# knagrecha/saturn

Measured on AMD Instinct MI355X. Metric: samples_per_s, higher is better.
Workload: dtype bf16; 1 GPU; model=gptj-6b, global_batch=16, seq_len=512, parallelism=dp1, optimizer=fused_sgd

## Files before the change

### saturn_amd/models/gptj.py

```python

from __future__ import annotations


from dataclasses import dataclass

import torch
import torch.nn as nn

from saturn_amd.ops.functional import (
    fused_gelu,
    FusedLayerNorm,
    apply_rope,
    causal_attention,
    fused_add3,
    fused_cross_entropy,
    rope_tables,
    FusedDropout,
    FusedEmbedding,
)


@dataclass
class GPTJConfig:
    vocab_size: int = 50400
    n_ctx: int = 512
    n_embd: int = 4096
    n_head: int = 16
    n_layer: int = 28
    rotary_dim: int = 64
    embd_pdrop: float = 0.0
    resid_pdrop: float = 0.0


class GPTJAttention(nn.Module):
    def __init__(self, cfg: GPTJConfig):
        super().__init__()
        self.n_head = cfg.n_head
        self.head_dim = cfg.n_embd // cfg.n_head
        self.rotary_dim = cfg.rotary_dim
        E = cfg.n_embd
        self.q_proj = nn.Linear(E, E, bias=False)
        self.k_proj = nn.Linear(E, E, bias=False)
        self.v_proj = nn.Linear(E, E, bias=False)
        self.out_proj = nn.Linear(E, E, bias=False)
        self.n_ctx = cfg.n_ctx
        self._rope_f32 = rope_tables(cfg.n_ctx, cfg.rotary_dim)

    def _rope(self, device):
        if self._rope_f32[0].device != device:
            self._rope_f32 = tuple(t.to(device) for t in self._rope_f32)
        return self._rope_f32

    def forward(self, x):
        B, T, E = x.shape
        H, D = self.n_head, self.head_dim
        q = self.q_proj(x).view(B, T, H, D)
        k = self.k_proj(x).view(B, T, H, D)
        v = self.v_proj(x).view(B, T, H, D)
        cos, sin = self._rope(x.device)
        q = apply_rope(q, cos, sin)
        k = apply_rope(k, cos, sin)
        q = q.transpose(1, 2)
        k = k.transpose(1, 2)
        v = v.transpose(1, 2)
        o = causal_attention(q, k, v)
        o = o.transpose(1, 2).reshape(B, T, -1)
        return self.out_proj(o)


class GPTJMLP(nn.Module):
    def __init__(self, cfg: GPTJConfig):
        super().__init__()
        E = cfg.n_embd
        self.fc_in = nn.Linear(E, 4 * E)
        self.fc_out = nn.Linear(4 * E, E)

    def forward(self, x):
        return self.fc_out(fused_gelu(self.fc_in(x)))


class GPTJBlock(nn.Module):

    def __init__(self, cfg: GPTJConfig):
        super().__init__()
        self.ln_1 = FusedLayerNorm(cfg.n_embd)
        self.attn = GPTJAttention(cfg)
        self.mlp = GPTJMLP(cfg)
        self.drop = FusedDropout(cfg.resid_pdrop)

    def forward(self, x):
        h = self.ln_1(x)
        return fused_add3(x, self.drop(self.attn(h)), self.drop(self.mlp(h)))


class GPTJForCausalLM(nn.Module):
    def __init__(self, cfg: GPTJConfig):
        super().__init__()
        self.cfg = cfg
        self.wte = FusedEmbedding(cfg.vocab_size, cfg.n_embd)
        self.drop = FusedDropout(cfg.embd_pdrop)
        self.h = nn.ModuleList(GPTJBlock(cfg) for _ in range(cfg.n_layer))
        self.ln_f = FusedLayerNorm(cfg.n_embd)
        self.lm_head = nn.Linear(cfg.n_embd, cfg.vocab_size, bias=True)
        self.apply(self._init)

    @staticmethod
    def _init(m):
        if isinstance(m, nn.Linear):
            nn.init.normal_(m.weight, std=0.02)
            if m.bias is not None:
                nn.init.zeros_(m.bias)
        elif isinstance(m, nn.Embedding):
            nn.init.normal_(m.weight, std=0.02)

    def forward(self, input_ids):
        x = self.drop(self.wte(input_ids))
        for block in self.h:
            x = block(x)
        x = self.ln_f(x)
        return self.lm_head(x)


def pretraining_loss(logits, labels):
    return fused_cross_entropy(logits, labels, shift=True)


class _EmbedStage(nn.Module):
    def __init__(self, wte):
        super().__init__()
        self.wte = wte

    def forward(self, input_ids):
        return self.wte(input_ids)


class _HeadStage(nn.Module):
    def __init__(self, ln_f, lm_head):
        super().__init__()
        self.ln_f = ln_f
        self.lm_head = lm_head

    def forward(self, x):
        return self.lm_head(self.ln_f(x))


def as_sequential(model: GPTJForCausalLM) -> nn.Sequential:
    return nn.Sequential(
        _EmbedStage(model.wte), *model.h, _HeadStage(model.ln_f, model.lm_head)
    )


def get_gptj_model(kwargs=None):
    kwargs = kwargs or {}
    cfg = GPTJConfig(
        n_layer=kwargs.get("n_layer", 28),
        n_embd=kwargs.get("n_embd", 4096),
        n_head=kwargs.get("n_head", 16),
        n_ctx=kwargs.get("n_ctx", 512),
        vocab_size=kwargs.get("vocab_size", 50400),
        rotary_dim=kwargs.get("rotary_dim", 64),
        embd_pdrop=kwargs.get("embd_pdrop", 0.0),
        resid_pdrop=kwargs.get("resid_pdrop", 0.0),
    )
    torch.manual_seed(kwargs.get("seed", 0))
    return GPTJForCausalLM(cfg)


class SyntheticTokens(torch.utils.data.Dataset):

    def __init__(self, n: int, seq_len: int, vocab: int, seed: int = 1):
        g = torch.Generator().manual_seed(seed)
        self.data = torch.randint(0, vocab, (n, seq_len), generator=g)

    def __len__(self):
        return len(self.data)

    def __getitem__(self, i):
        return self.data[i]


def _collate(batch):
    x = torch.stack(batch)
    return x, x.clone()


def make_token_dataloader(batch_size=8, seq_len=512, vocab=50400, n_batches=64):
    def get_dataloader():
        return torch.utils.data.DataLoader(
            SyntheticTokens(batch_size * n_batches, seq_len, vocab),
            batch_size=batch_size,
            shuffle=False,
            collate_fn=_collate,
        )

    return get_dataloader
```

### saturn_amd/ops/csrc/bindings.cpp

```cpp

#include <torch/extension.h>
#include <vector>

namespace samd {
void fused_sgd(std::vector<at::Tensor> params, std::vector<at::Tensor> grads,
               std::vector<at::Tensor> moms, std::vector<at::Tensor> masters,
               double lr, double momentum, double weight_decay);
void fused_adam(std::vector<at::Tensor> params, std::vector<at::Tensor> grads,
                std::vector<at::Tensor> ms, std::vector<at::Tensor> vs,
                std::vector<at::Tensor> masters, double lr, double beta1,
                double beta2, double eps, double weight_decay, double bc1,
                double bc2);
std::vector<at::Tensor> norm_fwd(at::Tensor x, at::Tensor w,
                                 c10::optional<at::Tensor> b, double eps,
                                 bool rms);
std::vector<at::Tensor> norm_bwd(at::Tensor dy, at::Tensor x, at::Tensor w,
                                 at::Tensor mean, at::Tensor rstd, bool rms,
                                 bool needs_db);
std::vector<at::Tensor> ce_fwd(at::Tensor logits, at::Tensor targets,
                               int64_t Tr, int64_t ignore_index);
at::Tensor ce_bwd(at::Tensor logits, at::Tensor targets, at::Tensor lse,
                  at::Tensor dloss, int64_t Tr, int64_t ignore_index);
void rope_apply(at::Tensor y, at::Tensor x, at::Tensor cos_t, at::Tensor sin_t,
                int64_t t_len, int64_t t_off, bool half_style, bool backward);
at::Tensor gelu_fwd(at::Tensor x);
at::Tensor gelu_bwd(at::Tensor dy, at::Tensor x);
std::vector<at::Tensor> attn_fwd(at::Tensor q, at::Tensor k, at::Tensor v,
                                 bool causal, int64_t kv_len);
std::vector<at::Tensor> attn_bwd(at::Tensor dout, at::Tensor q, at::Tensor k,
                                 at::Tensor v, at::Tensor o, at::Tensor lse,
                                 bool causal, int64_t kv_len);
at::Tensor add3(at::Tensor a, at::Tensor b, at::Tensor c);
at::Tensor swiglu_fwd(at::Tensor gate, at::Tensor up);
std::vector<at::Tensor> swiglu_bwd(at::Tensor dout, at::Tensor gate,
                                   at::Tensor up);
at::Tensor embed_fwd(at::Tensor weight, at::Tensor idx);
at::Tensor embed_bwd(at::Tensor dout, at::Tensor idx, long vocab);
at::Tensor dropout_fwd(at::Tensor x, double p, long seed);
at::Tensor dropout_bwd(at::Tensor dout, double p, long seed);
std::vector<at::Tensor> moe_route_fwd(at::Tensor logits, int64_t top_k,
                                      at::ScalarType out_dtype);
at::Tensor moe_route_bwd(at::Tensor logits, at::Tensor ids,
                         at::Tensor dweights);
std::vector<at::Tensor> moe_sort(at::Tensor ids, int64_t n_expert);
at::Tensor moe_permute_fwd(at::Tensor x, at::Tensor order, int64_t top_k);
at::Tensor moe_permute_bwd(at::Tensor dxs, at::Tensor pos);
at::Tensor moe_combine_fwd(at::Tensor y, at::Tensor weights, at::Tensor pos);
std::vector<at::Tensor> moe_combine_bwd(at::Tensor dout, at::Tensor y,
                                        at::Tensor weights, at::Tensor pos);
}

PYBIND11_MODULE(TORCH_EXTENSION_NAME, m) {
  m.doc() = "saturn_amd hand-written CDNA4 (gfx950) kernels";
  m.def("fused_sgd", &samd::fused_sgd, "fused multi-tensor SGD");
  m.def("fused_adam", &samd::fused_adam, "fused multi-tensor AdamW");
  m.def("norm_fwd", &samd::norm_fwd, "LayerNorm/RMSNorm forward");
  m.def("norm_bwd", &samd::norm_bwd, "LayerNorm/RMSNorm backward");
  m.def("ce_fwd", &samd::ce_fwd, "fused cross-entropy forward");
  m.def("ce_bwd", &samd::ce_bwd, "fused cross-entropy backward");
  m.def("rope_apply", &samd::rope_apply,
        "fused rotary embedding (out-of-place, offset table rows)");
  m.def("gelu_fwd", &samd::gelu_fwd, "fused tanh-approx GELU forward");
  m.def("gelu_bwd", &samd::gelu_bwd, "fused tanh-approx GELU backward");
  m.def("attn_fwd", &samd::attn_fwd, "fused flash attention forward",
        py::arg("q"), py::arg("k"), py::arg("v"), py::arg("causal"),
        py::arg("kv_len") = -1);
  m.def("attn_bwd", &samd::attn_bwd, "fused flash attention backward",
        py::arg("dout"), py::arg("q"), py::arg("k"), py::arg("v"),
        py::arg("o"), py::arg("lse"), py::arg("causal"),
        py::arg("kv_len") = -1);
  m.def("add3", &samd::add3, "fused 3-way residual add");
  m.def("swiglu_fwd", &samd::swiglu_fwd, "fused silu(gate)*up");
  m.def("swiglu_bwd", &samd::swiglu_bwd, "fused SwiGLU backward");
  m.def("embed_fwd", &samd::embed_fwd, "token embedding gather");
  m.def("embed_bwd", &samd::embed_bwd, "embedding scatter-add backward");
  m.def("dropout_fwd", &samd::dropout_fwd, "counter-based fused dropout");
  m.def("dropout_bwd", &samd::dropout_bwd, "dropout backward (mask recompute)");
  m.def("moe_route_fwd", &samd::moe_route_fwd,
        "MoE softmax + top-k + renormalise (ties to the lower expert)");
  m.def("moe_route_bwd", &samd::moe_route_bwd, "MoE routing backward");
  m.def("moe_sort", &samd::moe_sort,
        "stable counting sort of (token, slot) pairs by expert");
  m.def("moe_permute_fwd", &samd::moe_permute_fwd,
        "gather token rows into expert order");
  m.def("moe_permute_bwd", &samd::moe_permute_bwd,
        "sum each token's k permuted rows");
  m.def("moe_combine_fwd", &samd::moe_combine_fwd,
        "weighted sum of each token's k expert rows");
  m.def("moe_combine_bwd", &samd::moe_combine_bwd,
        "combine backward: dy and fp32 dweights");
}
```

### saturn_amd/ops/csrc/gelu.hip

```cpp

#include <torch/extension.h>
#include <ATen/hip/HIPContext.h>

#include "common.h"

namespace samd {

typedef __attribute__((ext_vector_type(8))) short short8v_g;

__device__ __forceinline__ float tanh_fast(float u) {
  return 1.f - 2.f / (__expf(2.f * u) + 1.f);
}

constexpr float GK = 0.7978845608028654f;
constexpr float GC = 0.044715f;

__device__ __forceinline__ float gelu_f(float x) {
  const float t = tanh_fast(GK * (x + GC * x * x * x));
  return 0.5f * x * (1.f + t);
}

__device__ __forceinline__ float dgelu_f(float x) {
  const float u = GK * (x + GC * x * x * x);
  const float t = tanh_fast(u);
  const float du = GK * (1.f + 3.f * GC * x * x);
  return 0.5f * (1.f + t) + 0.5f * x * (1.f - t * t) * du;
}

template <typename T, bool BWD>
__global__ void gelu_kernel(const T* __restrict__ x, const T* __restrict__ dy,
                            T* __restrict__ out, long n) {
  const long nv = n / 8;
  const long stride = (long)gridDim.x * blockDim.x;
  for (long i = blockIdx.x * (long)blockDim.x + threadIdx.x; i < nv;
       i += stride) {
    const short8v_g xv = *reinterpret_cast<const short8v_g*>(x + i * 8);
    short8v_g dv;
    if (BWD) dv = *reinterpret_cast<const short8v_g*>(dy + i * 8);
    short8v_g ov;
#pragma unroll
    for (int e = 0; e < 8; ++e) {
      T xe;
      xe.x = (unsigned short)xv[e];
      const float xf = toF<T>(xe);
      float r;
      if (BWD) {
        T de;
        de.x = (unsigned short)dv[e];
        r = toF<T>(de) * dgelu_f(xf);
      } else {
        r = gelu_f(xf);
      }
      ov[e] = (short)fromF<T>(r).x;
    }
    *reinterpret_cast<short8v_g*>(out + i * 8) = ov;
  }
  const long i0 = blockIdx.x * (long)blockDim.x + threadIdx.x;
  if (i0 == 0) {
    for (long j = nv * 8; j < n; ++j) {
      const float xf = toF<T>(x[j]);
      out[j] = fromF<T>(BWD ? toF<T>(dy[j]) * dgelu_f(xf) : gelu_f(xf));
    }
  }
}

static dim3 grid_1d(long work) {
  const int block = 256;
  return dim3((unsigned)std::max<long>(
      1, std::min<long>((work + block - 1) / block, 8192)));
}

at::Tensor gelu_fwd(at::Tensor x) {
  TORCH_CHECK(x.is_cuda() && x.is_contiguous());
  auto y = at::empty_like(x);
  const long n = x.numel();
  auto stream = at::hip::getCurrentHIPStream();
  AT_DISPATCH_FLOATING_TYPES_AND2(
      at::kBFloat16, at::kHalf, x.scalar_type(), "gelu_fwd", [&] {
        TORCH_CHECK(sizeof(scalar_t) == 2, "gelu kernel: 16-bit dtypes only");
        if constexpr (sizeof(scalar_t) == 2) {
          hipLaunchKernelGGL((gelu_kernel<scalar_t, false>), grid_1d(n / 8),
                             dim3(256), 0, stream.stream(),
                             reinterpret_cast<const scalar_t*>(x.data_ptr()),
                             (const scalar_t*)nullptr,
                             reinterpret_cast<scalar_t*>(y.data_ptr()), n);
        }
      });
  return y;
}

at::Tensor gelu_bwd(at::Tensor dy, at::Tensor x) {
  TORCH_CHECK(x.is_cuda() && x.is_contiguous() && dy.is_contiguous());
  TORCH_CHECK(dy.sizes() == x.sizes() && dy.scalar_type() == x.scalar_type());
  auto dx = at::empty_like(x);
  const long n = x.numel();
  auto stream = at::hip::getCurrentHIPStream();
  AT_DISPATCH_FLOATING_TYPES_AND2(
      at::kBFloat16, at::kHalf, x.scalar_type(), "gelu_bwd", [&] {
        TORCH_CHECK(sizeof(scalar_t) == 2, "gelu kernel: 16-bit dtypes only");
        if constexpr (sizeof(scalar_t) == 2) {
          hipLaunchKernelGGL((gelu_kernel<scalar_t, true>), grid_1d(n / 8),
                             dim3(256), 0, stream.stream(),
                             reinterpret_cast<const scalar_t*>(x.data_ptr()),
                             reinterpret_cast<const scalar_t*>(dy.data_ptr()),
                             reinterpret_cast<scalar_t*>(dx.data_ptr()), n);
        }
      });
  return dx;
}

}
```

### saturn_amd/ops/functional.py

```python

from __future__ import annotations

from typing import Tuple

import torch
import torch.nn.functional as F

from saturn_amd.ops import require_ext


class _NormFn(torch.autograd.Function):
    @staticmethod
    def forward(ctx, x, w, b, eps, rms):
        ext = require_ext()
        x = x.contiguous()
        y, mean, rstd = ext.norm_fwd(x, w, b, eps, rms)
        if rms:
            mean = rstd
        ctx.save_for_backward(x, w, mean, rstd)
        ctx.rms = rms
        ctx.has_b = b is not None
        return y

    @staticmethod
    def backward(ctx, dy):
        ext = require_ext()
        x, w, mean, rstd = ctx.saved_tensors
        dx, dw, db = ext.norm_bwd(
            dy.contiguous(), x, w, mean, rstd, ctx.rms, ctx.has_b
        )
        return (
            dx,
            dw.to(w.dtype),
            db.to(w.dtype) if ctx.has_b else None,
            None,
            None,
        )


def fused_layer_norm(x, weight, bias=None, eps: float = 1e-5):
    if x.is_cuda:
        return _NormFn.apply(x, weight, bias, eps, False)
    return F.layer_norm(
        x.float(), (x.shape[-1],),
        weight.float(), bias.float() if bias is not None else None, eps
    ).to(x.dtype)


def fused_rms_norm(x, weight, eps: float = 1e-6):
    if x.is_cuda:
        return _NormFn.apply(x, weight, None, eps, True)
    xf = x.float()
    y = xf * torch.rsqrt(xf.pow(2).mean(-1, keepdim=True) + eps)
    return (y * weight.float()).to(x.dtype)


class FusedLayerNorm(torch.nn.Module):
    def __init__(self, dim: int, eps: float = 1e-5, bias: bool = True):
        super().__init__()
        self.eps = eps
        self.weight = torch.nn.Parameter(torch.ones(dim))
        self.bias = torch.nn.Parameter(torch.zeros(dim)) if bias else None

    def forward(self, x):
        return fused_layer_norm(x, self.weight, self.bias, self.eps)


class FusedRMSNorm(torch.nn.Module):
    def __init__(self, dim: int, eps: float = 1e-6):
        super().__init__()
        self.eps = eps
        self.weight = torch.nn.Parameter(torch.ones(dim))

    def forward(self, x):
        return fused_rms_norm(x, self.weight, self.eps)


class _CeFn(torch.autograd.Function):
    @staticmethod
    def forward(ctx, logits, targets_flat, Tr, ignore_index):
        ext = require_ext()
        loss, lse = ext.ce_fwd(logits, targets_flat, Tr, ignore_index)
        valid = (targets_flat != ignore_index).sum().clamp(min=1)
        ctx.save_for_backward(logits, targets_flat, lse, valid)
        ctx.Tr = Tr
        ctx.ignore_index = ignore_index
        return loss.sum() / valid.float()

    @staticmethod
    def backward(ctx, grad_out):
        ext = require_ext()
        logits, targets_flat, lse, valid = ctx.saved_tensors
        dloss = torch.full_like(lse, 0.0)
        dloss.fill_(1.0)
        dloss = dloss * (grad_out.float() / valid.float())
        dlogits = ext.ce_bwd(
            logits, targets_flat, lse, dloss, ctx.Tr, ctx.ignore_index
        )
        return dlogits, None, None, None


def fused_cross_entropy(
    logits: torch.Tensor,
    targets: torch.Tensor,
    shift: bool = True,
    ignore_index: int = -100,
) -> torch.Tensor:
    B, T, V = logits.shape
    if logits.is_cuda:
        Tr = T - 1 if shift else T
        tg = targets[:, 1:] if shift else targets
        return _CeFn.apply(
            logits.contiguous(), tg.contiguous().view(-1), Tr, ignore_index
        )
    if shift:
        lg = logits[:, :-1].float().reshape(-1, V)
        tg = targets[:, 1:].reshape(-1)
    else:
        lg = logits.float().reshape(-1, V)
        tg = targets.reshape(-1)
    return F.cross_entropy(lg, tg, ignore_index=ignore_index)


def rope_tables(
    T: int,
    rotary_dim: int,
    base: float = 10000.0,
    device=None,
    interleaved: bool = True,
) -> Tuple[torch.Tensor, torch.Tensor]:
    half = rotary_dim // 2
    inv = 1.0 / (base ** (torch.arange(0, half, dtype=torch.float32) * 2 / rotary_dim))
    t = torch.arange(T, dtype=torch.float32)
    freqs = torch.outer(t, inv)
    return freqs.cos().to(device), freqs.sin().to(device)


class _RopeFn(torch.autograd.Function):
    @staticmethod
    def forward(ctx, x, cos_t, sin_t, t_len, t_off, half_style):
        ext = require_ext()
        x = x.contiguous()
        y = torch.empty_like(x)
        ext.rope_apply(y, x, cos_t, sin_t, t_len, t_off, half_style, False)
        ctx.save_for_backward(cos_t, sin_t)
        ctx.meta = (t_len, t_off, half_style)
        return y

    @staticmethod
    def backward(ctx, dy):
        ext = require_ext()
        cos_t, sin_t = ctx.saved_tensors
        t_len, t_off, half_style = ctx.meta
        dy = dy.contiguous()
        dx = torch.empty_like(dy)
        ext.rope_apply(dx, dy, cos_t, sin_t, t_len, t_off, half_style, True)
        return dx, None, None, None, None, None


def _rope_cpu(x, cos_bt, sin_bt, half_style):
    B, T, H, D = x.shape
    half = cos_bt.shape[-1]
    c = cos_bt.view(B, T, 1, half).float()
    s = sin_bt.view(B, T, 1, half).float()
    xf = x.float()
    out = xf.clone()
    if half_style:
        x0 = xf[..., :half]
        x1 = xf[..., half : 2 * half]
        out[..., :half] = x0 * c - x1 * s
        out[..., half : 2 * half] = x1 * c + x0 * s
    else:
        x0 = xf[..., 0 : 2 * half : 2]
        x1 = xf[..., 1 : 2 * half : 2]
        out[..., 0 : 2 * half : 2] = x0 * c - x1 * s
        out[..., 1 : 2 * half : 2] = x1 * c + x0 * s
    return out.to(x.dtype)


def apply_rope(
    x: torch.Tensor,
    cos: torch.Tensor,
    sin: torch.Tensor,
    half_style: bool = False,
) -> torch.Tensor:
    B, T, H, D = x.shape
    half = cos.shape[-1]
    from saturn_amd.parallel.sequence import _STATE as _sp

    off = _sp["rank"] * T if _sp["world"] > 1 else 0
    if cos.shape[0] < off + T:
        raise ValueError(
            "rope table too short for this sequence shard — pass the FULL "
            "table to apply_rope (it slices positions itself)"
        )
    if cos.dtype != torch.float32:
        cos = cos.float()
        sin = sin.float()
    if x.is_cuda:
        return _RopeFn.apply(x, cos.contiguous(), sin.contiguous(), T, off,
                             half_style)
    cos_bt = cos[off : off + T].unsqueeze(0).expand(B, T, half)
    sin_bt = sin[off : off + T].unsqueeze(0).expand(B, T, half)
    return _rope_cpu(x, cos_bt.contiguous(), sin_bt.contiguous(), half_style)


def attention_math(q, k, v, causal: bool = True) -> torch.Tensor:
    scale = 1.0 / (q.shape[-1] ** 0.5)
    s = torch.matmul(q.float(), k.float().transpose(-1, -2)) * scale
    if causal:
        T = q.shape[-2]
        mask = torch.ones(T, T, dtype=torch.bool, device=q.device).tril()
        s = s.masked_fill(~mask, float("-inf"))
    p = torch.softmax(s, dim=-1)
    return torch.matmul(p, v.float()).to(q.dtype)


def _attention_core(q, k, v, causal: bool) -> torch.Tensor:
    if q.is_cuda:
        from saturn_amd.ops import flash

        return flash.flash_attention(q, k, v, causal=causal)
    if k.shape[1] != q.shape[1]:
        rep = q.shape[1] // k.shape[1]
        k = k.repeat_interleave(rep, dim=1)
        v = v.repeat_interleave(rep, dim=1)
    return attention_math(q, k, v, causal=causal)


def _attention(q, k, v, causal: bool) -> torch.Tensor:
    from saturn_amd.parallel.sequence import sp_attention, sp_world

    if sp_world() > 1:
        return sp_attention(q, k, v, lambda a, b, c: _attention_core(a, b, c, causal))
    return _attention_core(q, k, v, causal)


def causal_attention(q, k, v) -> torch.Tensor:
    return _attention(q, k, v, causal=True)


def full_attention(q, k, v) -> torch.Tensor:
    return _attention(q, k, v, causal=False)


class _Add3Fn(torch.autograd.Function):
    @staticmethod
    def forward(ctx, a, b, c):
        ext = require_ext()
        return ext.add3(a.contiguous(), b.contiguous(), c.contiguous())

    @staticmethod
    def backward(ctx, g):
        return g, g, g


def fused_add3(a, b, c):
    if a.is_cuda:
        return _Add3Fn.apply(a, b, c)
    return a + b + c


class _GeluFn(torch.autograd.Function):
    @staticmethod
    def forward(ctx, x):
        ext = require_ext()
        x = x.contiguous()
        ctx.save_for_backward(x)
        return ext.gelu_fwd(x)

    @staticmethod
    def backward(ctx, dy):
        ext = require_ext()
        (x,) = ctx.saved_tensors
        return ext.gelu_bwd(dy.contiguous(), x)


def fused_gelu(x: torch.Tensor) -> torch.Tensor:
    if x.is_cuda and x.dtype in (torch.bfloat16, torch.float16):
        return _GeluFn.apply(x)
    return torch.nn.functional.gelu(x, approximate="tanh")


class _SwigluFn(torch.autograd.Function):
    @staticmethod
    def forward(ctx, gate, up):
        ext = require_ext()
        gate = gate.contiguous()
        up = up.contiguous()
        ctx.save_for_backward(gate, up)
        return ext.swiglu_fwd(gate, up)

    @staticmethod
    def backward(ctx, dout):
        ext = require_ext()
        gate, up = ctx.saved_tensors
        dgate, dup = ext.swiglu_bwd(dout.contiguous(), gate, up)
        return dgate, dup


def fused_swiglu(gate, up):
    if gate.is_cuda:
        return _SwigluFn.apply(gate, up)
    return torch.nn.functional.silu(gate) * up


class _EmbedFn(torch.autograd.Function):
    @staticmethod
    def forward(ctx, weight, idx):
        ext = require_ext()
        ctx.save_for_backward(idx)
        ctx.vocab = weight.shape[0]
        return ext.embed_fwd(weight, idx)

    @staticmethod
    def backward(ctx, dout):
        ext = require_ext()
        (idx,) = ctx.saved_tensors
        return ext.embed_bwd(dout, idx, ctx.vocab), None


def fused_embedding(weight, idx):
    if weight.is_cuda:
        return _EmbedFn.apply(weight, idx)
    return F.embedding(idx, weight)


class FusedEmbedding(torch.nn.Embedding):

    def forward(self, idx):
        if (
            self.weight.is_cuda
            and self.padding_idx is None
            and self.max_norm is None
            and not self.sparse
            and self.weight.dtype
            in (torch.bfloat16, torch.float16, torch.float32)
        ):
            return _EmbedFn.apply(self.weight, idx)
        return super().forward(idx)


class _DropoutFn(torch.autograd.Function):
    @staticmethod
    def forward(ctx, x, p, seed):
        ext = require_ext()
        ctx.p = p
        ctx.seed = seed
        return ext.dropout_fwd(x, p, seed)

    @staticmethod
    def backward(ctx, dout):
        ext = require_ext()
        return ext.dropout_bwd(dout.contiguous(), ctx.p, ctx.seed), None, None


def fused_dropout(x, p: float, training: bool = True):
    if p == 0.0 or not training:
        return x
    if x.is_cuda and x.dtype in (torch.bfloat16, torch.float16):
        seed = int(torch.randint(0, 2**62, (1,)).item())
        return _DropoutFn.apply(x.contiguous(), p, seed)
    return F.dropout(x, p, training)


class FusedDropout(torch.nn.Module):
    def __init__(self, p: float = 0.0):
        super().__init__()
        self.p = p

    def forward(self, x):
        return fused_dropout(x, self.p, self.training)

    def extra_repr(self):
        return f"p={self.p}"
```

### setup.py

```python

import os

from setuptools import setup

os.environ.setdefault("PYTORCH_ROCM_ARCH", "gfx950")

from torch.utils.cpp_extension import BuildExtension, CUDAExtension

CSRC = os.path.join("saturn_amd", "ops", "csrc")

ext = CUDAExtension(
    name="saturn_amd._C",
    sources=[
        os.path.join(CSRC, "bindings.cpp"),
        os.path.join(CSRC, "fused_optim.hip"),
        os.path.join(CSRC, "layernorm.hip"),
        os.path.join(CSRC, "cross_entropy.hip"),
        os.path.join(CSRC, "rope.hip"),
        os.path.join(CSRC, "gelu.hip"),
        os.path.join(CSRC, "attention.hip"),
        os.path.join(CSRC, "add3.hip"),
        os.path.join(CSRC, "swiglu.hip"),
        os.path.join(CSRC, "embedding.hip"),
        os.path.join(CSRC, "dropout.hip"),
        os.path.join(CSRC, "moe.hip"),
    ],
    extra_compile_args={
        "cxx": ["-O3", "-std=c++17"],
        "nvcc": ["-O3", "-std=c++17", "--offload-arch=gfx950"],
    },
)

comm_ext = CUDAExtension(
    name="saturn_amd._comm",
    sources=[os.path.join("saturn_amd", "comm", "csrc", "rccl_comm.cpp")],
    libraries=["rccl"],
    extra_compile_args={
        "cxx": ["-O3", "-std=c++17"],
        "nvcc": ["-O3", "-std=c++17", "--offload-arch=gfx950"],
    },
)

setup(
    name="saturn_amd",
    version="0.1.0",
    packages=[
        "saturn_amd",
        "saturn_amd.core",
        "saturn_amd.library",
        "saturn_amd.solver",
        "saturn_amd.engine",
        "saturn_amd.trial_runner",
        "saturn_amd.executors",
        "saturn_amd.parallel",
        "saturn_amd.ops",
        "saturn_amd.comm",
        "saturn_amd.models",
        "saturn_amd.utils",
    ],
    ext_modules=[ext, comm_ext],
    cmdclass={"build_ext": BuildExtension},
)
```

Measured before the change: 59.41 samples/s.

## Add fused GPT-J MLP backward with TN-layout weight gradients and fused bias sums

Adds a custom autograd function for the GPT-J MLP. Its backward fuses the GELU derivative with a transposed copy of d_pre and of gelu(pre), and computes the column sums for the bias gradients in the same pass. The transposed operands let the weight-gradient GEMMs run in a TN layout, which is meant to be a faster path for hipBLASLt than the transposed-A mm calls autograd would issue. It also stops saving the GELU output in forward and recomputes it in backward, which saves activation memory. The cost is extra transpose traffic and more temporary buffers.

New measurement: 61.70 samples/s (median of 6 runs). +3.9%, better.

```diff
diff --git a/saturn_amd/models/gptj.py b/saturn_amd/models/gptj.py
--- a/saturn_amd/models/gptj.py
+++ b/saturn_amd/models/gptj.py
@@ -2,6 +2,7 @@
 from __future__ import annotations
 
 
+import os
 from dataclasses import dataclass
 
 import torch
@@ -17,6 +18,8 @@
     rope_tables,
     FusedDropout,
     FusedEmbedding,
+    gptj_mlp,
+    mlp_fused_supported,
 )
 
 
@@ -75,7 +78,30 @@
         self.fc_in = nn.Linear(E, 4 * E)
         self.fc_out = nn.Linear(4 * E, E)
 
-    def forward(self, x):
+    @staticmethod
+    def _plain_linear(m) -> bool:
+        return type(m) is nn.Linear and not (
+            m._forward_hooks
+            or m._forward_pre_hooks
+            or m._backward_hooks
+            or m._backward_pre_hooks
+        )
+
+    def _use_fused(self, x) -> bool:
+        if os.environ.get("SAMD_MLP_FUSED", "1") == "0":
+            return False
+        fi, fo = self.fc_in, self.fc_out
+        return (
+            x.is_cuda
+            and self._plain_linear(fi)
+            and self._plain_linear(fo)
+            and mlp_fused_supported(x, fi.weight, fi.bias, fo.weight, fo.bias)
+        )
+
+    def forward(self, x):
+        if self._use_fused(x):
+            fi, fo = self.fc_in, self.fc_out
+            return gptj_mlp(x, fi.weight, fi.bias, fo.weight, fo.bias)
         return self.fc_out(fused_gelu(self.fc_in(x)))
 
 
diff --git a/saturn_amd/ops/csrc/bindings.cpp b/saturn_amd/ops/csrc/bindings.cpp
--- a/saturn_amd/ops/csrc/bindings.cpp
+++ b/saturn_amd/ops/csrc/bindings.cpp
@@ -48,6 +48,12 @@
 at::Tensor moe_combine_fwd(at::Tensor y, at::Tensor weights, at::Tensor pos);
 std::vector<at::Tensor> moe_combine_bwd(at::Tensor dout, at::Tensor y,
                                         at::Tensor weights, at::Tensor pos);
+std::vector<at::Tensor> mlp_act_bwd(at::Tensor d_act, at::Tensor pre,
+                                    bool want_dT, bool want_aT);
+std::vector<at::Tensor> transpose_colsum(at::Tensor x, bool want_sum);
+std::vector<at::Tensor> mlp_bwd(at::Tensor g, at::Tensor h, at::Tensor pre,
+                                at::Tensor W_in, at::Tensor W_out,
+                                bool use_tn_in, bool use_tn_out);
 }
 
 PYBIND11_MODULE(TORCH_EXTENSION_NAME, m) {
@@ -89,4 +95,12 @@
         "weighted sum of each token's k expert rows");
   m.def("moe_combine_bwd", &samd::moe_combine_bwd,
         "combine backward: dy and fp32 dweights");
+  m.def("mlp_act_bwd", &samd::mlp_act_bwd,
+        "GELU backward + transposed d_pre / gelu(pre) + fp32 bias grad",
+        py::arg("d_act"), py::arg("pre"), py::arg("want_dT") = true,
+        py::arg("want_aT") = true);
+  m.def("transpose_colsum", &samd::transpose_colsum,
+        "bf16 transpose with optional fp32 column sums");
+  m.def("mlp_bwd", &samd::mlp_bwd,
+        "GPT-J MLP backward with TN-layout weight gradients");
 }
diff --git a/saturn_amd/ops/csrc/gelu.hip b/saturn_amd/ops/csrc/gelu.hip
--- a/saturn_amd/ops/csrc/gelu.hip
+++ b/saturn_amd/ops/csrc/gelu.hip
@@ -3,29 +3,11 @@
 #include <ATen/hip/HIPContext.h>
 
 #include "common.h"
+#include "gelu_math.h"
 
 namespace samd {
 
 typedef __attribute__((ext_vector_type(8))) short short8v_g;
-
-__device__ __forceinline__ float tanh_fast(float u) {
-  return 1.f - 2.f / (__expf(2.f * u) + 1.f);
-}
-
-constexpr float GK = 0.7978845608028654f;
-constexpr float GC = 0.044715f;
-
-__device__ __forceinline__ float gelu_f(float x) {
-  const float t = tanh_fast(GK * (x + GC * x * x * x));
-  return 0.5f * x * (1.f + t);
-}
-
-__device__ __forceinline__ float dgelu_f(float x) {
-  const float u = GK * (x + GC * x * x * x);
-  const float t = tanh_fast(u);
-  const float du = GK * (1.f + 3.f * GC * x * x);
-  return 0.5f * (1.f + t) + 0.5f * x * (1.f - t * t) * du;
-}
 
 template <typename T, bool BWD>
 __global__ void gelu_kernel(const T* __restrict__ x, const T* __restrict__ dy,
diff --git a/saturn_amd/ops/csrc/gelu_math.h b/saturn_amd/ops/csrc/gelu_math.h
--- /dev/null
+++ b/saturn_amd/ops/csrc/gelu_math.h
@@ -0,0 +1,26 @@
+#pragma once
+
+#include <hip/hip_runtime.h>
+
+namespace samd {
+
+__device__ __forceinline__ float tanh_fast(float u) {
+  return 1.f - 2.f / (__expf(2.f * u) + 1.f);
+}
+
+constexpr float GK = 0.7978845608028654f;
+constexpr float GC = 0.044715f;
+
+__device__ __forceinline__ float gelu_f(float x) {
+  const float t = tanh_fast(GK * (x + GC * x * x * x));
+  return 0.5f * x * (1.f + t);
+}
+
+__device__ __forceinline__ float dgelu_f(float x) {
+  const float u = GK * (x + GC * x * x * x);
+  const float t = tanh_fast(u);
+  const float du = GK * (1.f + 3.f * GC * x * x);
+  return 0.5f * (1.f + t) + 0.5f * x * (1.f - t * t) * du;
+}
+
+}
diff --git a/saturn_amd/ops/csrc/mlp_bwd.hip b/saturn_amd/ops/csrc/mlp_bwd.hip
--- /dev/null
+++ b/saturn_amd/ops/csrc/mlp_bwd.hip
@@ -0,0 +1,334 @@
+
+#include <torch/extension.h>
+#include <ATen/hip/HIPContext.h>
+
+#include "common.h"
+#include "gelu_math.h"
+
+namespace samd {
+
+namespace {
+
+constexpr int MB_TILE = 64;
+constexpr int MB_ROW_ITERS = 4;
+constexpr int MB_BLOCK = 256;
+
+typedef c10::BFloat16 bf16_t;
+
+__device__ __forceinline__ int img_dword(int c, int rp) {
+  return c * 32 + (((rp >> 2) ^ (c >> 3)) << 2) + (rp & 3);
+}
+__device__ __forceinline__ int img_slot(int c, int mv) {
+  return c * 8 + (mv ^ (c >> 3));
+}
+
+__device__ __forceinline__ float sum8_bf16(const uint4 v) {
+  float s = us2f((unsigned short)(v.x & 0xffffu));
+  s += us2f((unsigned short)(v.x >> 16));
+  s += us2f((unsigned short)(v.y & 0xffffu));
+  s += us2f((unsigned short)(v.y >> 16));
+  s += us2f((unsigned short)(v.z & 0xffffu));
+  s += us2f((unsigned short)(v.z >> 16));
+  s += us2f((unsigned short)(v.w & 0xffffu));
+  s += us2f((unsigned short)(v.w >> 16));
+  return s;
+}
+
+__device__ __forceinline__ void store_colsums(float acc0, float acc1,
+                                              float4* lds_sum,
+                                              float* __restrict__ partial,
+                                              long col0, long ncols) {
+  const int tid = threadIdx.x;
+#pragma unroll
+  for (int off = 1; off < 8; off <<= 1) {
+    acc0 += __shfl_xor(acc0, off, 64);
+    acc1 += __shfl_xor(acc1, off, 64);
+  }
+  float* s = reinterpret_cast<float*>(lds_sum);
+  if ((tid & 7) == 0) {
+    s[tid >> 3] = acc0;
+    s[(tid >> 3) + 32] = acc1;
+  }
+  __syncthreads();
+  if (tid < MB_TILE / 4 && col0 + tid * 4 < ncols) {
+    *reinterpret_cast<float4*>(partial + (long)blockIdx.y * ncols + col0 +
+                               tid * 4) = lds_sum[tid];
+  }
+}
+
+template <bool TN_IN, bool TN_OUT>
+__global__ void __launch_bounds__(MB_BLOCK)
+mlp_act_bwd_kernel(const bf16_t* __restrict__ d_act,
+                   const bf16_t* __restrict__ pre, bf16_t* __restrict__ d_pre,
+                   bf16_t* __restrict__ d_preT, bf16_t* __restrict__ act,
+                   float* __restrict__ partial, long M, long F) {
+  __shared__ uint4 img_d[MB_TILE * 8];
+  __shared__ uint4 img_a[TN_OUT ? MB_TILE * 8 : 1];
+  __shared__ float4 lds_sum[MB_TILE / 4];
+
+  const int tid = threadIdx.x;
+  const int cv = tid & 7;
+  const int rp = tid >> 3;
+  const int mv = tid & 7;
+  const int cr = tid >> 3;
+  const long col0 = (long)blockIdx.x * MB_TILE;
+  const long col = col0 + cv * 8;
+  const bool col_ok = col < F;
+
+  float acc0 = 0.f, acc1 = 0.f;
+
+  for (int it = 0; it < MB_ROW_ITERS; ++it) {
+    const long row0 = ((long)blockIdx.y * MB_ROW_ITERS + it) * MB_TILE;
+    if (row0 >= M) break;
+    const long row = row0 + 2 * rp;
+    const bool ok = col_ok && row < M;
+
+    const short8v zero8 = {0, 0, 0, 0, 0, 0, 0, 0};
+    short8v xv[2], gv[2];
+#pragma unroll
+    for (int i = 0; i < 2; ++i) {
+      if (ok) {
+        const long o = (row + i) * F + col;
+        xv[i] = *reinterpret_cast<const short8v*>(pre + o);
+        gv[i] = *reinterpret_cast<const short8v*>(d_act + o);
+      } else {
+        xv[i] = zero8;
+        gv[i] = zero8;
+      }
+    }
+    short8v dv[2], av[2];
+#pragma unroll
+    for (int i = 0; i < 2; ++i) {
+#pragma unroll
+      for (int e = 0; e < 8; ++e) {
+        bf16_t xe, de;
+        xe.x = (unsigned short)xv[i][e];
+        de.x = (unsigned short)gv[i][e];
+        const float xf = toF<bf16_t>(xe);
+        dv[i][e] = (short)fromF<bf16_t>(toF<bf16_t>(de) * dgelu_f(xf)).x;
+        av[i][e] = (short)fromF<bf16_t>(gelu_f(xf)).x;
+      }
+    }
+    if (ok) {
+#pragma unroll
+      for (int i = 0; i < 2; ++i) {
+        const long o = (row + i) * F + col;
+        *reinterpret_cast<short8v*>(d_pre + o) = dv[i];
+        if (!TN_OUT) *reinterpret_cast<short8v*>(act + o) = av[i];
+      }
+    }
+    unsigned* d32 = reinterpret_cast<unsigned*>(img_d);
+    unsigned* a32 = reinterpret_cast<unsigned*>(img_a);
+#pragma unroll
+    for (int e = 0; e < 8; ++e) {
+      const int w = img_dword(cv * 8 + e, rp);
+      d32[w] = ok ? ((unsigned)(unsigned short)dv[0][e] |
+                     ((unsigned)(unsigned short)dv[1][e] << 16))
+                  : 0u;
+      if (TN_OUT)
+        a32[w] = ok ? ((unsigned)(unsigned short)av[0][e] |
+                       ((unsigned)(unsigned short)av[1][e] << 16))
+                    : 0u;
+    }
+    __syncthreads();
+
+    const long mrow = row0 + mv * 8;
+#pragma unroll
+    for (int j = 0; j < 2; ++j) {
+      const int c = cr + 32 * j;
+      const uint4 d = img_d[img_slot(c, mv)];
+      const float s = sum8_bf16(d);
+      if (j == 0) acc0 += s; else acc1 += s;
+      const bool st = (col0 + c < F) && (mrow < M);
+      if (TN_IN && st)
+        *reinterpret_cast<uint4*>(d_preT + (col0 + c) * M + mrow) = d;
+      if (TN_OUT && st)
+        *reinterpret_cast<uint4*>(act + (col0 + c) * M + mrow) =
+            img_a[img_slot(c, mv)];
+    }
+    __syncthreads();
+  }
+  store_colsums(acc0, acc1, lds_sum, partial, col0, F);
+}
+
+template <bool SUM, bool STORE>
+__global__ void __launch_bounds__(MB_BLOCK)
+transpose_colsum_kernel(const bf16_t* __restrict__ x, bf16_t* __restrict__ xT,
+                        float* __restrict__ partial, long M, long N) {
+  __shared__ uint4 img[MB_TILE * 8];
+  __shared__ float4 lds_sum[MB_TILE / 4];
+
+  const int tid = threadIdx.x;
+  const int cv = tid & 7;
+  const int rp = tid >> 3;
+  const int mv = tid & 7;
+  const int cr = tid >> 3;
+  const long col0 = (long)blockIdx.x * MB_TILE;
+  const long col = col0 + cv * 8;
+  const bool col_ok = col < N;
+
+  float acc0 = 0.f, acc1 = 0.f;
+
+  for (int it = 0; it < MB_ROW_ITERS; ++it) {
+    const long row0 = ((long)blockIdx.y * MB_ROW_ITERS + it) * MB_TILE;
+    if (row0 >= M) break;
+    const long row = row0 + 2 * rp;
+    const bool ok = col_ok && row < M;
+
+    const short8v zero8 = {0, 0, 0, 0, 0, 0, 0, 0};
+    short8v xv[2];
+#pragma unroll
+    for (int i = 0; i < 2; ++i) {
+      xv[i] = zero8;
+      if (ok) xv[i] = *reinterpret_cast<const short8v*>(x + (row + i) * N + col);
+    }
+    unsigned* i32 = reinterpret_cast<unsigned*>(img);
+#pragma unroll
+    for (int e = 0; e < 8; ++e) {
+      i32[img_dword(cv * 8 + e, rp)] =
+          (unsigned)(unsigned short)xv[0][e] |
+          ((unsigned)(unsigned short)xv[1][e] << 16);
+    }
+    __syncthreads();
+
+    const long mrow = row0 + mv * 8;
+#pragma unroll
+    for (int j = 0; j < 2; ++j) {
+      const int c = cr + 32 * j;
+      const uint4 v = img[img_slot(c, mv)];
+      if (SUM) {
+        const float s = sum8_bf16(v);
+        if (j == 0) acc0 += s; else acc1 += s;
+      }
+      if (STORE && (col0 + c < N) && (mrow < M))
+        *reinterpret_cast<uint4*>(xT + (col0 + c) * M + mrow) = v;
+    }
+    __syncthreads();
+  }
+  if (SUM) store_colsums(acc0, acc1, lds_sum, partial, col0, N);
+}
+
+void check_operand(const at::Tensor& t, const char* name) {
+  TORCH_CHECK(t.is_cuda(), name, ": expected a GPU tensor");
+  TORCH_CHECK(t.scalar_type() == at::kBFloat16, name, ": expected bf16");
+  TORCH_CHECK(t.dim() == 2 && t.is_contiguous(), name,
+              ": expected a contiguous 2-D tensor");
+  TORCH_CHECK(t.size(0) > 0 && t.size(0) % 8 == 0 && t.size(1) > 0 &&
+                  t.size(1) % 8 == 0,
+              name, ": both sizes must be positive multiples of 8, got ",
+              t.sizes());
+  TORCH_CHECK(reinterpret_cast<uintptr_t>(t.data_ptr()) % 16 == 0, name,
+              ": data must be 16-byte aligned");
+}
+
+dim3 tile_grid(long M, long N) {
+  const long gx = (N + MB_TILE - 1) / MB_TILE;
+  const long gy = (M + MB_TILE * MB_ROW_ITERS - 1) / (MB_TILE * MB_ROW_ITERS);
+  TORCH_CHECK(gy <= 65535, "mlp_bwd: too many rows for one launch");
+  return dim3((unsigned)gx, (unsigned)gy);
+}
+
+bf16_t* bptr(const at::Tensor& t) {
+  return reinterpret_cast<bf16_t*>(t.data_ptr());
+}
+
+}
+
+std::vector<at::Tensor> mlp_act_bwd(at::Tensor d_act, at::Tensor pre,
+                                    bool want_dT, bool want_aT) {
+  check_operand(d_act, "mlp_act_bwd d_act");
+  check_operand(pre, "mlp_act_bwd pre");
+  TORCH_CHECK(d_act.sizes() == pre.sizes(), "mlp_act_bwd: shape mismatch");
+  const long M = pre.size(0), F = pre.size(1);
+  auto d_pre = at::empty_like(pre);
+  auto d_preT = want_dT ? at::empty({F, M}, pre.options())
+                        : at::empty({0}, pre.options());
+  auto act = want_aT ? at::empty({F, M}, pre.options()) : at::empty_like(pre);
+  const dim3 grid = tile_grid(M, F);
+  auto partial =
+      at::empty({(long)grid.y, F}, pre.options().dtype(at::kFloat));
+  auto stream = at::hip::getCurrentHIPStream();
+#define SAMD_LAUNCH_ACT_BWD(TI, TO)                                        \
+  hipLaunchKernelGGL((mlp_act_bwd_kernel<TI, TO>), grid, dim3(MB_BLOCK), 0, \
+                     stream.stream(), bptr(d_act), bptr(pre), bptr(d_pre),  \
+                     want_dT ? bptr(d_preT) : nullptr, bptr(act),           \
+                     partial.data_ptr<float>(), M, F)
+  if (want_dT && want_aT) SAMD_LAUNCH_ACT_BWD(true, true);
+  else if (want_dT) SAMD_LAUNCH_ACT_BWD(true, false);
+  else if (want_aT) SAMD_LAUNCH_ACT_BWD(false, true);
+  else SAMD_LAUNCH_ACT_BWD(false, false);
+#undef SAMD_LAUNCH_ACT_BWD
+  SAMD_CHECK_HIP(hipGetLastError());
+  return {d_pre, d_preT, act, at::sum(partial, {0})};
+}
+
+namespace {
+
+std::vector<at::Tensor> transpose_colsum_impl(const at::Tensor& x,
+                                              bool want_sum, bool want_store) {
+  check_operand(x, "transpose_colsum x");
+  TORCH_CHECK(want_sum || want_store, "transpose_colsum: nothing to do");
+  const long M = x.size(0), N = x.size(1);
+  auto xT = want_store ? at::empty({N, M}, x.options())
+                       : at::empty({0}, x.options());
+  const dim3 grid = tile_grid(M, N);
+  const auto fopt = x.options().dtype(at::kFloat);
+  auto partial = want_sum ? at::empty({(long)grid.y, N}, fopt)
+                          : at::empty({0}, fopt);
+  auto stream = at::hip::getCurrentHIPStream();
+#define SAMD_LAUNCH_TRANSPOSE(SUM, STORE)                                    \
+  hipLaunchKernelGGL((transpose_colsum_kernel<SUM, STORE>), grid,            \
+                     dim3(MB_BLOCK), 0, stream.stream(), bptr(x),            \
+                     want_store ? bptr(xT) : nullptr,                        \
+                     want_sum ? partial.data_ptr<float>() : nullptr, M, N)
+  if (want_sum && want_store) SAMD_LAUNCH_TRANSPOSE(true, true);
+  else if (want_sum) SAMD_LAUNCH_TRANSPOSE(true, false);
+  else SAMD_LAUNCH_TRANSPOSE(false, true);
+#undef SAMD_LAUNCH_TRANSPOSE
+  SAMD_CHECK_HIP(hipGetLastError());
+  return {xT, want_sum ? at::sum(partial, {0}) : partial};
+}
+
+}
+
+std::vector<at::Tensor> transpose_colsum(at::Tensor x, bool want_sum) {
+  return transpose_colsum_impl(x, want_sum, true);
+}
+
+std::vector<at::Tensor> mlp_bwd(at::Tensor g, at::Tensor h, at::Tensor pre,
+                                at::Tensor W_in, at::Tensor W_out,
+                                bool use_tn_in, bool use_tn_out) {
+  check_operand(g, "mlp_bwd g");
+  check_operand(h, "mlp_bwd h");
+  check_operand(pre, "mlp_bwd pre");
+  check_operand(W_in, "mlp_bwd W_in");
+  check_operand(W_out, "mlp_bwd W_out");
+  const long M = g.size(0), E = g.size(1), F = pre.size(1);
+  TORCH_CHECK(h.size(0) == M && h.size(1) == E && pre.size(0) == M &&
+                  W_in.size(0) == F && W_in.size(1) == E &&
+                  W_out.size(0) == E && W_out.size(1) == F,
+              "mlp_bwd: inconsistent shapes");
+
+  at::Tensor d_pre, d_preT, act, db_in;
+  {
+    auto d_act = at::mm(g, W_out);
+    auto r = mlp_act_bwd(d_act, pre, use_tn_in, use_tn_out);
+    d_pre = r[0];
+    d_preT = r[1];
+    act = r[2];
+    db_in = r[3];
+  }
+  auto gt = transpose_colsum_impl(g, true, use_tn_out);
+  at::Tensor hT;
+  if (use_tn_in) hT = transpose_colsum_impl(h, false, true)[0];
+  auto dW_out = use_tn_out ? at::linear(gt[0], act) : at::mm(g.t(), act);
+  act.reset();
+  auto dW_in = use_tn_in ? at::linear(d_preT, hT) : at::mm(d_pre.t(), h);
+  d_preT.reset();
+  hT.reset();
+  auto dh = at::mm(d_pre, W_in);
+  return {dh, dW_in, db_in.to(W_in.scalar_type()), dW_out,
+          gt[1].to(W_out.scalar_type())};
+}
+
+}
diff --git a/saturn_amd/ops/functional.py b/saturn_amd/ops/functional.py
--- a/saturn_amd/ops/functional.py
+++ b/saturn_amd/ops/functional.py
@@ -1,6 +1,7 @@
 
 from __future__ import annotations
 
+import os
 from typing import Tuple
 
 import torch
@@ -282,6 +283,66 @@
     return torch.nn.functional.gelu(x, approximate="tanh")
 
 
+_MLP_TN_DEFAULT = {"in": True, "out": True}
+
+
+def _mlp_tn(site: str) -> bool:
+    v = os.environ.get("SAMD_MLP_TN_" + site.upper())
+    return _MLP_TN_DEFAULT[site] if v is None else v != "0"
+
+
+def mlp_fused_supported(x, w_in, b_in, w_out, b_out) -> bool:
+    if not (x.is_cuda and x.dtype == torch.bfloat16 and x.dim() >= 2):
+        return False
+    if b_in is None or b_out is None:
+        return False
+    if any(t.dtype != torch.bfloat16 or not t.is_cuda
+           for t in (w_in, b_in, w_out, b_out)):
+        return False
+    E = x.shape[-1]
+    M = x.numel() // E if E else 0
+    F_ = w_in.shape[0]
+    return (
+        M > 0
+        and w_in.shape == (F_, E)
+        and w_out.shape == (E, F_)
+        and M % 8 == 0
+        and E % 8 == 0
+        and F_ % 8 == 0
+    )
+
+
+class _GPTJMlpFn(torch.autograd.Function):
+
+    @staticmethod
+    def forward(ctx, h, w_in, b_in, w_out, b_out):
+        ext = require_ext()
+        pre = F.linear(h, w_in, b_in).contiguous()
+        out = F.linear(ext.gelu_fwd(pre), w_out, b_out)
+        ctx.save_for_backward(h, pre, w_in, w_out)
+        return out
+
+    @staticmethod
+    def backward(ctx, g):
+        ext = require_ext()
+        h, pre, w_in, w_out = ctx.saved_tensors
+        E = h.shape[-1]
+        dh, dw_in, db_in, dw_out, db_out = ext.mlp_bwd(
+            g.contiguous().view(-1, E),
+            h.contiguous().view(-1, E),
+            pre.view(-1, pre.shape[-1]),
+            w_in.contiguous(),
+            w_out.contiguous(),
+            _mlp_tn("in"),
+            _mlp_tn("out"),
+        )
+        return dh.view(h.shape), dw_in, db_in, dw_out, db_out
+
+
+def gptj_mlp(h, w_in, b_in, w_out, b_out):
+    return _GPTJMlpFn.apply(h, w_in, b_in, w_out, b_out)
+
+
 class _SwigluFn(torch.autograd.Function):
     @staticmethod
     def forward(ctx, gate, up):
diff --git a/setup.py b/setup.py
--- a/setup.py
+++ b/setup.py
@@ -24,6 +24,7 @@
         os.path.join(CSRC, "embedding.hip"),
         os.path.join(CSRC, "dropout.hip"),
         os.path.join(CSRC, "moe.hip"),
+        os.path.join(CSRC, "mlp_bwd.hip"),
     ],
     extra_compile_args={
         "cxx": ["-O3", "-std=c++17"],
```
